# VachaLab/gorder

Measured on AMD Instinct MI355X. Metric: trajectory frames/sec, higher is better.
Workload: dtype f32

## Files before the change

gorder_amd/csrc/gorder_hip.hip:

```cpp
#include <hip/hip_runtime.h>

#include <dlfcn.h>

#include <cmath>
#include <cstdio>
#include <cstdlib>
#include <cstring>
#include <mutex>
#include <new>
#include <string>
#include <deque>
#include <type_traits>
#include <vector>

#include "../../include/gorder_hip.h"
#include "gm_math.h"
#include "plan.h"
#include "collect_store.h"
#include "replay_rows.h"
#include "timewise_blocks.h"
#include "ordermap_final.h"
#include "order_route.h"

#pragma clang fp contract(off)

using gorder::DirectItem;
using gorder::Item;
using gorder::kBlock;
using gorder::Plan;
using gorder::Tile;

#include "kernels_common.h"
#include "kernels_bonds.h"
#include "kernels_extras.h"
#include "kernels_radial.h"
#include "kernels_leaflets.h"
#include "kernels_cluster.h"
#include "kernels_cluster_cutoff.h"
#include "kernels_normals.h"
#include "kernels_xtc.h"
#include "kernels_trr.h"
#include "kernels_collect.h"
#include "kernels_replay.h"
#include "kernels_timewise.h"
#include "kernels_ordermap.h"


struct gorder_hip_handle {
    void *traj_cache = nullptr;
    void (*traj_cache_free)(gorder_hip_handle *) = nullptr;
    Plan plan;
    gorder_tables_t tables{};
    int device = 0;
    hipStream_t own_stream = nullptr;
    hipStream_t stream = nullptr;
// ... 1775 lines not shown
        HIP_TRY(h, hipMalloc((void **)&nc, ncap * row * sizeof(unsigned long long)));
        HIP_TRY(h, hipMemsetAsync(ns, 0, ncap * row * sizeof(unsigned long long), h->stream));
        HIP_TRY(h, hipMemsetAsync(nc, 0, ncap * row * sizeof(unsigned long long), h->stream));
        if (h->d_tw_sums) {
            HIP_TRY(h, hipMemcpyAsync(ns, h->d_tw_sums, h->n_frames * row * sizeof(unsigned long long), hipMemcpyDeviceToDevice, h->stream));
            HIP_TRY(h, hipMemcpyAsync(nc, h->d_tw_cnts, h->n_frames * row * sizeof(unsigned long long), hipMemcpyDeviceToDevice, h->stream));
            HIP_TRY(h, hipStreamSynchronize(h->stream));
            HIP_TRY(h, hipFree(h->d_tw_sums));
            HIP_TRY(h, hipFree(h->d_tw_cnts));
        }
        h->d_tw_sums = ns; h->d_tw_cnts = nc; h->tw_cap = ncap;
    }
    FrameArgs a{};
    a.xyz = d_xyz; a.box9 = d_box; a.n_atoms = p.n_atoms; a.n_frames = n_frames;
    a.pbc = pbc ? 1 : 0;
    a.nx = h->tables.normal[0]; a.ny = h->tables.normal[1]; a.nz = h->tables.normal[2]; a.n2 = h->n2; a.n2sq = h->n2sq;
    a.leaflets = leaflets ? 1 : 0; a.aflags = h->d_aflags; a.arow = h->d_arow; a.n_mol_total = p.n_mol_total;
    a.acc = h->d_acc; a.rep = h->d_rep; a.n_rep = h->n_rep; a.n_acc = p.n_acc; a.err = h->d_err;
    h->manual_active = false;
    if (h->manual_frames) {
        const size_t n4 = (size_t)n_frames * p.n_mol_total;
        if ((st = ensure(h, &h->d_dyn_normals, &h->dyn_normals_cap, n4)) != GORDER_OK) return abort_batch(st);
        if (hipStreamSynchronize(h->stream) != hipSuccess ||
            hipMemcpy(h->d_dyn_normals, h->manual_normals.data(), n4 * 4 * sizeof(float), hipMemcpyHostToDevice) != hipSuccess)
            return abort_batch(fail(h, GORDER_ERR_DEVICE, "manual normals: copy to the device failed"));
        h->manual_active = true;
        h->manual_frames = 0;
    } else if (h->d_ntable) {
        if ((st = replay_normal_rows(h, normal_rows)) != GORDER_OK) return abort_batch(st);
        h->manual_active = true;
    }
    const uint32_t n_tiles_all = (uint32_t)p.tiles.size();
    if (spec) {
        if ((st = ensure(h, &h->d_mom, &h->mom_cap, (size_t)n_frames * n_tiles_all)) != GORDER_OK) return abort_batch(st);
        if ((st = ensure(h, &h->d_head_z, &h->head_z_cap, (size_t)n_frames * p.n_mol_total)) != GORDER_OK) return abort_batch(st);
        a.own = h->d_own; a.mom = h->d_mom; a.mom_dim = (int)lf.normal_dim;
        a.own_head_begin = h->d_own_head_begin; a.own_heads = h->d_own_heads; a.head_z = h->d_head_z;
    }
    h->extra.touched = nullptr;
    if ((h->collect & GORDER_COLLECT_NORMALS) && h->extra.geom_kind && !p.tiles.empty() && p.ua_tiles.empty()) {
        const size_t nt = (size_t)n_frames * p.n_mol_total;
        if ((st = ensure(h, &h->d_touched, &h->touched_cap, nt)) != GORDER_OK) return abort_batch(st);
        if (hipMemsetAsync(h->d_touched, 0, nt, h->stream) != hipSuccess) return abort_batch(fail(h, GORDER_ERR_DEVICE, "collect: hipMemsetAsync"));
        h->extra.touched = h->d_touched;
    }
    st = launch_orders(h, a, route);
    h->manual_active = false;
    if (st != GORDER_OK) return abort_batch(st);
    h->rep_dirty = true;
    if (spec) {
        size_t cap_c = h->spec_frames_cap, cap_o = h->spec_frames_cap;
        if ((st = ensure(h, &h->d_spec_center, &cap_c, n_frames)) != GORDER_OK) return abort_batch(st);
        if ((st = ensure(h, &h->d_spec_ok, &cap_o, n_frames)) != GORDER_OK) return abort_batch(st);
        h->spec_frames_cap = std::min(cap_c, cap_o);
        uint32_t *cnt = h->d_spec_counters + 2u * (uint32_t)(h->spec_batches & 1u);
        uint32_t *cnt_next = h->d_spec_counters + 2u * (uint32_t)((h->spec_batches + 1u) & 1u);
        SpecArgs sa{};
        sa.xyz = d_xyz; sa.box9 = d_box; sa.n_atoms = p.n_atoms; sa.n_frames = n_frames; sa.n_tiles = n_tiles_all;
        sa.n_mol_total = p.n_mol_total; sa.n_membrane = lf.n_membrane; sa.dim = lf.normal_dim; sa.flip = lf.flip ? 1 : 0;
        sa.pbc = pbc ? 1 : 0; sa.mom = h->d_mom; sa.head_z = h->d_head_z; sa.center = h->d_spec_center; sa.ok = h->d_spec_ok;
        sa.aflags = h->d_aflags; sa.adist = h->d_adist; sa.counters = cnt; sa.counters_next = cnt_next;
        const uint32_t ring_slot = (uint32_t)(h->spec_batches % gorder_hip_handle::kSpecRing);
        sa.host_counters = h->h_spec_counters + 2u * ring_slot; sa.err = h->d_err;
        (void)timing_mark(h, "k_spec_check + k_spec_fixup");
        hipLaunchKernelGGL(k_spec_check, dim3(std::min<uint32_t>(n_frames, 2048u)), dim3(256), 0, h->stream, sa);
        if ((st = run_leaflets(h, d_xyz, d_box, spec_aframes, 1, h->d_spec_ok)) != GORDER_OK) return abort_batch(st);
        (void)timing_mark(h, "k_spec_check + k_spec_fixup");
        const uint32_t fix_grid = (uint32_t)std::min<uint64_t>(((uint64_t)n_frames * p.n_mol_total + 63u) / 64u, 4096u);
        with_bool(route.fixup_ac, [&](auto AC) { with_bool(route.fixup_tw, [&](auto TW) {
            if constexpr (!AC() || !TW())
                hipLaunchKernelGGL((k_spec_fixup<AC(), TW()>), dim3(fix_grid), dim3(64), 0, h->stream, a, sa, h->d_spec_mol_begin,
                                   h->d_spec_samples, TW() ? h->d_tw_sums : nullptr, TW() ? h->d_tw_cnts : nullptr,
                                   TW() ? (uint64_t)h->n_frames : (uint64_t)0);
        }); });
        hipLaunchKernelGGL(k_spec_finish, dim3(1), dim3(256), 0, h->stream, sa);
        HIP_TRY(h, hipGetLastError());
        HIP_TRY(h, hipEventRecord(h->spec_counters_copied[ring_slot], h->stream));
        h->spec_ring_frames[ring_slot] = n_frames;
        h->spec_batches++;
    }
    if ((st = collect_flag_rows(h, 1, collect_frames)) != GORDER_OK) return abort_batch(st);
    if (ltable && (h->collect & GORDER_COLLECT_LEAFLETS)) {
        for (size_t k = 0; k < replay.collect_rows.size();) {
            size_t e = k + 1;
            while (e < replay.collect_rows.size() && replay.collect_rows[e] == replay.collect_rows[e - 1] + 1u) e++;
            const std::vector<uint64_t> run(replay.collect_frames.begin() + k, replay.collect_frames.begin() + e);
            if ((st = collect_flag_rows(h, replay.collect_rows[k], run)) != GORDER_OK) return abort_batch(st);
            k = e;
        }
    }
    if ((h->collect & GORDER_COLLECT_NORMALS) && p.n_mol_total && !h->d_ntable &&
        (st = collect_normal_rows(h, frame_index, n_frames, h->extra.touched)) != GORDER_OK) return abort_batch(st);
    if (n_new_rows) {
        HIP_TRY(h, hipMemcpyAsync(h->d_aflags, h->d_aflags + n_new_rows * (size_t)p.n_mol_total, p.n_mol_total,
                                  hipMemcpyDeviceToDevice, h->stream));
    }
    if (ltable) { h->replay_have_carry = replay.have_carry; h->replay_carry_index = replay.carry_index; }
    {
// ... 906 lines not shown
```

gorder_amd/csrc/kernels_bonds.h:

```cpp
#pragma once

namespace {

__device__ __forceinline__ int grid_index(float x, float lo, float bin, uint32_t n, bool core) {
    const float k = __builtin_roundf(core ? gm_div_core(x - lo, bin) : (x - lo) / bin);
    if (!(k >= 0.0f) || !(k < (float)n)) return -1;
    return (int)k;
}
__device__ __forceinline__ int grid_index_fast(float x, float lo, float inv_bin, uint32_t n) {
    const float k = __builtin_floorf(__builtin_fmaf(x - lo, inv_bin, 0.5f));
    if (!(k >= 0.0f) || !(k < (float)n)) return -1;
    return (int)k;
}
constexpr uint32_t kRecFrames = 4;
struct TiledMapOut {
    uint32_t plane;
    float x0, y0, binx, biny;
    uint32_t nx, ny;
    int bin_core;
    unsigned long long *words;
    unsigned long long *ticks;
};
__device__ __forceinline__ unsigned long long tick_sample_word(int tick, bool lower) {
    return ((unsigned long long)(lower ? 1u : 0u) << 32) | (unsigned long long)(uint32_t)tick;
// ... 82 lines not shown
    }
    template <bool TAIL, bool FINITE = false>
    static __device__ __forceinline__ bool store(const FrameArgs &a, const Tile &t, uint32_t f0, uint32_t f_end,
                                                 uint32_t sk, uint32_t si, const v4f (&pre)[NPF], float *lds,
                                                 uint32_t lw) {
        const uint32_t f = f0 + sk;
        if (TAIL && f >= f_end) return true;
        const size_t base = ((size_t)f * a.n_atoms + t.atom0) * 3u;
        const uint32_t n4 = ((uint32_t)(base & 3u) + 3u * t.n_window + 3u) >> 2;
        const v4f *src = reinterpret_cast<const v4f *>(a.xyz + (base & ~(size_t)3));
        v4f *dst = reinterpret_cast<v4f *>(lds + (size_t)sk * lw);
        typedef float v2f __attribute__((ext_vector_type(2)));
        v2f poison = {0.0f, 0.0f};
        const v2f zero2 = {0.0f, 0.0f};
#pragma unroll
        for (int j = 0; j < NPF; j++) {
            const uint32_t i = si + (uint32_t)j * TPF;
            if (i < n4) dst[i] = pre[j];
            if (FINITE) {
                poison = __builtin_elementwise_fma(pre[j].xy, zero2, poison);
                poison = __builtin_elementwise_fma(pre[j].zw, zero2, poison);
            }
        }
        for (uint32_t i = si + (uint32_t)NPF * TPF; i < n4; i += TPF) {
            const v4f v = __builtin_nontemporal_load(src + i);
            dst[i] = v;
            if (FINITE) {
                poison = __builtin_elementwise_fma(v.xy, zero2, poison);
                poison = __builtin_elementwise_fma(v.zw, zero2, poison);
            }
        }
        return poison.x + poison.y == 0.0f;
    }
    template <int NF, int OUT = 0>
    static __device__ __forceinline__ void compute_core(const FrameArgs &a, const Tile &t, const Item &it,
                                                        uint32_t f0, const float (&P)[NF][6], SampleAcc &acc,
                                                        int &bad, uint32_t &nan_which, uint32_t &nan_frame,
                                                        const TiledMapOut *mo = nullptr, uint32_t k0 = 0) {
        constexpr bool MAPS = OUT != 0;
        int tick[NF];
        uint8_t fl[NF];
        float bx[NF], by[NF], bz[NF];
        uint32_t rare = 0;
        auto stage_word = [&](int k, float vx, float vy, float vz) {
            mo->words[k0 + (uint32_t)k] = OUT == 2
                ? tick_sample_word(tick[k], LEAF && fl[k] != 0)
                : map_sample_word(*mo, P[k][0] + vx / 2.0f, P[k][1] + vy / 2.0f, P[k][2] + vz / 2.0f, tick[k], LEAF && fl[k] != 0);
            if (OUT == 3) mo->ticks[k0 + (uint32_t)k] = tick_sample_word(tick[k], LEAF && fl[k] != 0);
        };
#pragma unroll
        for (int k = 0; k < NF; k++) {
            if (PBC) {
                const float *b = a.box9 + 9 * (size_t)(f0 + k);
                bx[k] = b[0]; by[k] = b[4]; bz[k] = b[8];
            }
            if (LEAF) fl[k] = a.aflags[(size_t)a.arow[f0 + k] * a.n_mol_total + it.mol];
        }
#pragma unroll
        for (int k = 0; k < NF; k++) {
            float vx = P[k][3] - P[k][0], vy = P[k][4] - P[k][1], vz = P[k][5] - P[k][2];
            bool slow = false;
            if (PBC && AXIS >= 0 && !ACOS_COS && !MAPS) {
                const float ax = __builtin_fabsf(vx), ay = __builtin_fabsf(vy), az = __builtin_fabsf(vz);
                const float tx = bx[k] - ax, ty = by[k] - ay, tz = bz[k] - az;
                vx = ax > bx[k] / 2.0f ? tx : ax;
                vy = ay > by[k] / 2.0f ? ty : ay;
                vz = az > bz[k] / 2.0f ? tz : az;
                slow = __builtin_fminf(__builtin_fminf(tx, ty), tz) < 0.0f;
            } else if (PBC) {
                vx = gm_min_image_step(vx, bx[k], slow);
                vy = gm_min_image_step(vy, by[k], slow);
                vz = gm_min_image_step(vz, bz[k], slow);
            }
            if (AXIS >= 0 && !ACOS_COS) {
                const float sch = gm_sch_axis<AXIS>(vx, vy, vz, slow);
                rare |= (slow ? 1u : 0u) << k;
                tick[k] = gm_tick_finite(sch);
            } else if (AXIS >= 0) {
                const float sch = gm_sch_axis_acos<AXIS>(vx, vy, vz, slow);
                rare |= (slow ? 1u : 0u) << k;
                tick[k] = gm_tick_finite(sch);
            } else {
                bool nonfinite = false;
                const float sch = gm_calc_sch<ACOS_COS, AXIS>(vx, vy, vz, a.nx, a.ny, a.nz, a.n2, a.n2sq, &nonfinite);
                rare |= ((slow || nonfinite || sch != sch) ? 1u : 0u) << k;
                tick[k] = gm_tick(sch);
            }
            if (MAPS) stage_word(k, vx, vy, vz);
        }
        if (__builtin_expect(rare != 0, 0)) {
#pragma unroll
            for (int k = 0; k < NF; k++) {
                if (!((rare >> k) & 1u)) continue;
                float vx = P[k][3] - P[k][0], vy = P[k][4] - P[k][1], vz = P[k][5] - P[k][2];
                if (PBC) {
                    vx = gm_min_image_loop(vx, bx[k], bad);
                    vy = gm_min_image_loop(vy, by[k], bad);
                    vz = gm_min_image_loop(vz, bz[k], bad);
                }
                const float sch = gm_calc_sch<ACOS_COS>(vx, vy, vz, a.nx, a.ny, a.nz, a.n2, a.n2sq);
                tick[k] = gm_tick(sch);
                if (MAPS) stage_word(k, vx, vy, vz);
                if (sch != sch && nan_frame == kNoNan) {
                    if (P[k][0] != P[k][0]) { nan_which = 0; nan_frame = f0 + k; }
                    else if (P[k][3] != P[k][3]) { nan_which = 1; nan_frame = f0 + k; }
                }
            }
        }
        int st = 0, su = 0;
        uint32_t nu = 0;
#pragma unroll
        for (int k = 0; k < NF; k++) {
            st += tick[k];
            if (LEAF) {
                su += fl[k] == 0 ? tick[k] : 0;
                nu += fl[k] == 0 ? 1u : 0u;
            }
        }
        acc.s_tot += st;
        acc.n_tot += NF;
        acc.s_up += su;
        acc.n_up += nu;
    }
    template <int OUT = 0>
    static __device__ __forceinline__ void compute(const FrameArgs &a, const Tile &t, const Item &it, uint32_t f0,
                                                   const float *lds, uint32_t lw, SampleAcc &acc, int &bad,
                                                   uint32_t &nan_which, uint32_t &nan_frame, const TiledMapOut *mo = nullptr) {
        constexpr int NF = (OUT == 1 || OUT == 3 || (OUT == 2 && LEAF)) ? 2 : (GORDER_COMPUTE_NF < G ? GORDER_COMPUTE_NF : G);
#pragma unroll
        for (int h = 0; h < G; h += NF) {
            float P[NF][6];
#pragma unroll
            for (int k = 0; k < NF; k++) {
                const uint32_t sh = (uint32_t)((((size_t)(f0 + h + k) * a.n_atoms + t.atom0) * 3u) & 3u);
                const float *w = lds + (size_t)(h + k) * lw + sh;
                P[k][0] = w[3u * it.li]; P[k][1] = w[3u * it.li + 1]; P[k][2] = w[3u * it.li + 2];
                P[k][3] = w[3u * it.lj]; P[k][4] = w[3u * it.lj + 1]; P[k][5] = w[3u * it.lj + 2];
            }
            compute_core<NF, OUT>(a, t, it, f0 + h, P, acc, bad, nan_which, nan_frame, mo, (uint32_t)h);
        }
    }
    template <int OUT = 0>
    static __device__ __forceinline__ void compute_tail(const FrameArgs &a, const Tile &t, const Item &it,
                                                        uint32_t f0, uint32_t f_end, const float *lds, uint32_t lw,
                                                        SampleAcc &acc, int &bad, uint32_t &nan_which,
                                                        uint32_t &nan_frame, const TiledMapOut *mo = nullptr) {
        if (OUT != 0) {
#pragma unroll
            for (int k = 0; k < G; k++) {
                const uint32_t f = f0 + (uint32_t)k;
                if (f >= f_end) continue;
                const uint32_t sh = (uint32_t)((((size_t)f * a.n_atoms + t.atom0) * 3u) & 3u);
                const float *w = lds + (size_t)k * lw + sh;
                const float p1x = w[3u * it.li], p1y = w[3u * it.li + 1], p1z = w[3u * it.li + 2];
                const float p2x = w[3u * it.lj], p2y = w[3u * it.lj + 1], p2z = w[3u * it.lj + 2];
                if (bond_sample<ACOS_COS>(a, f, p1x, p1y, p1z, p2x, p2y, p2z, it.mol, acc, bad, mo, mo->words + k, OUT == 3 ? mo->ticks + k : nullptr) &&
                    nan_frame == kNoNan) {
                    if (p1x != p1x) { nan_which = 0; nan_frame = f; }
                    else if (p2x != p2x) { nan_which = 1; nan_frame = f; }
                }
            }
            return;
        }
#pragma unroll 1
        for (uint32_t f = f0; f < f_end; f++) {
            const uint32_t sh = (uint32_t)((((size_t)f * a.n_atoms + t.atom0) * 3u) & 3u);
            const float *w = lds + (size_t)(f - f0) * lw + sh;
            const float p1x = w[3u * it.li], p1y = w[3u * it.li + 1], p1z = w[3u * it.li + 2];
            const float p2x = w[3u * it.lj], p2y = w[3u * it.lj + 1], p2z = w[3u * it.lj + 2];
            if (bond_sample<ACOS_COS>(a, f, p1x, p1y, p1z, p2x, p2y, p2z, it.mol, acc, bad) && nan_frame == kNoNan) {
                if (p1x != p1x) { nan_which = 0; nan_frame = f; }
                else if (p2x != p2x) { nan_which = 1; nan_frame = f; }
            }
        }
    }
};

#ifndef GORDER_TILED_MIN_WAVES
#define GORDER_TILED_MIN_WAVES 4
#endif
__device__ __forceinline__ float mom_min(float x, float y) { float r; __asm__("v_min_f32_e32 %0, %1, %2" : "=v"(r) : "v"(x), "v"(y)); return r; }
__device__ __forceinline__ float mom_max(float x, float y) { float r; __asm__("v_max_f32_e32 %0, %1, %2" : "=v"(r) : "v"(x), "v"(y)); return r; }
#define GORDER_MOM_MINMAX_DPP(CTRL_TEXT)                                                                    \
    __asm__("s_nop 1\n\tv_min_f32_dpp %0, %0, %0 " CTRL_TEXT "\n\tv_max_f32_dpp %1, %1, %1 " CTRL_TEXT : "+v"(mn), "+v"(mx))
__device__ __forceinline__ void tiled_moments(const FrameArgs &a, const Tile &t, uint2 own, uint32_t tile_id, uint32_t n_tiles,
                                              uint32_t f, const float *slot, bool finite, uint2 my_head) {
    const uint32_t lane = threadIdx.x & 63u;
    const uint32_t sh = (uint32_t)((((size_t)f * a.n_atoms + t.atom0) * 3u) & 3u);
    const float *w = slot + sh + a.mom_dim + 3u * (own.x - t.atom0);
    const uint32_t n_own = own.y - own.x;
    float s = 0.0f, q = 0.0f, mn = 3.0e38f, mx = -3.0e38f;
    for (uint32_t i0 = 0; i0 < n_own; i0 += 512u) {
        float z[8];
#pragma unroll
        for (uint32_t u = 0; u < 8u; u++) z[u] = w[3u * min(i0 + 64u * u + lane, n_own - 1u)];
#pragma unroll
        for (uint32_t u = 0; u < 8u; u++) {
            if (i0 + 64u * u >= n_own) break;
            float d = z[u];
            if (i0 + 64u * u + 64u > n_own) d = i0 + 64u * u + lane < n_own ? d : 0.0f;
            s += d;
            q = __builtin_fmaf(d, d, q);
            mn = mom_min(mn, z[u]);
            mx = mom_max(mx, z[u]);
        }
    }
#define GORDER_MOM_STEP(CTRL, MASK, CTRL_TEXT)                                                  \
    s += dpp_or_zero<CTRL, MASK>(s); q += dpp_or_zero<CTRL, MASK>(q);                               \
    GORDER_MOM_MINMAX_DPP(CTRL_TEXT);
    GORDER_MOM_STEP(0x111, 0xf, "row_shr:1 row_mask:0xf bank_mask:0xf")
    GORDER_MOM_STEP(0x112, 0xf, "row_shr:2 row_mask:0xf bank_mask:0xf")
    GORDER_MOM_STEP(0x114, 0xf, "row_shr:4 row_mask:0xf bank_mask:0xf")
    GORDER_MOM_STEP(0x118, 0xf, "row_shr:8 row_mask:0xf bank_mask:0xf")
    GORDER_MOM_STEP(0x142, 0xa, "row_bcast:15 row_mask:0xa bank_mask:0xf")
    GORDER_MOM_STEP(0x143, 0xc, "row_bcast:31 row_mask:0xc bank_mask:0xf")
#undef GORDER_MOM_STEP
    const bool all_finite = __all(finite);
    if (lane == 63u) a.mom[(size_t)f * n_tiles + tile_id] = make_float4(all_finite ? s : __builtin_nanf(""), q, mn, mx);
    if (my_head.y != 0xffffffffu) a.head_z[(size_t)f * a.n_mol_total + my_head.y] = slot[sh + a.mom_dim + 3u * my_head.x];
}
template <int G, int NPF, bool ACOS_COS, bool PBC, bool LEAF, int AXIS, bool MOM = false>
__global__ __launch_bounds__(kBlock, GORDER_TILED_MIN_WAVES) void k_bonds_tiled(FrameArgs a_in, const float *__restrict__ xyz,
                                                      const float *__restrict__ box9,
                                                      const uint8_t *__restrict__ aflags,
                                                      const uint32_t *__restrict__ arow,
                                                      const Tile *__restrict__ tiles,
                                                      const Item *__restrict__ items,
                                                      const uint32_t *__restrict__ tile_slots,
                                                      uint32_t n_tiles, uint32_t lw) {
    extern __shared__ __attribute__((aligned(16))) float lds[];
    using S = TiledStage<G, NPF, ACOS_COS, PBC, LEAF, AXIS>;
    FrameArgs a = a_in;
    a.xyz = xyz; a.box9 = box9; a.aflags = aflags; a.arow = arow;
    const uint32_t tile_id = blockIdx.x % n_tiles;
    const uint32_t chunk = blockIdx.x / n_tiles;
    const Tile t = tiles[tile_id];
    const uint32_t tid = threadIdx.x;
    const uint32_t sk = tid / S::TPF, si = tid % S::TPF;
    const bool active = tid < t.n_items;
    Item it{0, 0, 0, 0, 0};
    if (active) it = items[t.item0 + tid];

    const uint32_t f_begin = chunk * a.frames_per_chunk;
    const uint32_t f_end = min(a.n_frames, f_begin + a.frames_per_chunk);
    const uint32_t f_full = f_begin + ((f_end - f_begin) / G) * G;

    SampleAcc acc;
    int bad = 0;
    uint32_t nan_which = 0, nan_frame = kNoNan;
    v4f pre[NPF];
    uint2 own = make_uint2(0u, 0u), my_head = make_uint2(0u, 0xffffffffu);
    if (MOM) {
        own = a.own[tile_id];
        const uint32_t hq = a.own_head_begin[tile_id] + (tid & 63u);
        if (hq < a.own_head_begin[tile_id + 1u]) my_head = a.own_heads[hq];
    }

    if (f_begin < f_full) S::template load<false>(a, t, f_begin, f_end, sk, si, pre);
    for (uint32_t f0 = f_begin; f0 < f_full; f0 += G) {
        const bool finite = S::template store<false, MOM>(a, t, f0, f_end, sk, si, pre, lds, lw);
        __syncthreads();
        if (f0 + G < f_full) S::template load<false>(a, t, f0 + G, f_end, sk, si, pre);
        if (MOM) {
            static_assert(!MOM || (uint32_t)G * 64u == kBlock, "a wave per frame slot");
            tiled_moments(a, t, own, tile_id, n_tiles, f0 + sk, lds + (size_t)sk * lw, finite, my_head);
        }
        if (active) S::compute(a, t, it, f0, lds, lw, acc, bad, nan_which, nan_frame);
        __syncthreads();
    }
    if (f_full < f_end) {
        S::template load<true>(a, t, f_full, f_end, sk, si, pre);
        const bool finite = S::template store<true, MOM>(a, t, f_full, f_end, sk, si, pre, lds, lw);
        __syncthreads();
        if (MOM && f_full + sk < f_end) tiled_moments(a, t, own, tile_id, n_tiles, f_full + sk, lds + (size_t)sk * lw, finite, my_head);
        if (active) S::compute_tail(a, t, it, f_full, f_end, lds, lw, acc, bad, nan_which, nan_frame);
        __syncthreads();
    }

    if (nan_frame != kNoNan)
        raise_error(a.err, GORDER_ERR_UNDEFINED_POSITION, nan_frame, kStageTypes, tile_slots[t.slot0 + it.lslot], 1, it.mol, nan_which);
    if (bad) raise_box_range(a.err, f_begin);

    unsigned long long *l_s = reinterpret_cast<unsigned long long *>(lds);
    uint32_t *l_n = reinterpret_cast<uint32_t *>(l_s + 2 * kBlock);
    l_s[tid] = 0; l_s[kBlock + tid] = 0; l_n[tid] = 0; l_n[kBlock + tid] = 0;
    __syncthreads();
    if (active && acc.n_tot) {
        atomicAdd(&l_s[it.lslot], (unsigned long long)acc.s_tot);
        atomicAdd(&l_n[it.lslot], acc.n_tot);
        if (acc.n_up) {
            atomicAdd(&l_s[kBlock + it.lslot], (unsigned long long)acc.s_up);
            atomicAdd(&l_n[kBlock + it.lslot], acc.n_up);
        }
    }
    __syncthreads();
#ifdef GORDER_DEBUG_NOEPILOGUE
    if (a.n_frames == 0xffffffffu)
#endif
    if (tid < t.n_slots && l_n[tid]) {
        unsigned long long *acc = a.rep + (size_t)(blockIdx.x % a.n_rep) * 4u * a.n_acc;
        const uint32_t slot = tile_slots[t.slot0 + tid];
        atomicAdd(&acc[slot], l_s[tid]);
        atomicAdd(&acc[2u * a.n_acc + slot], (unsigned long long)l_n[tid]);
        if (l_n[kBlock + tid]) {
            atomicAdd(&acc[a.n_acc + slot], l_s[kBlock + tid]);
            atomicAdd(&acc[3u * a.n_acc + slot], (unsigned long long)l_n[kBlock + tid]);
        }
// ... 128 lines not shown
```

gorder_amd/csrc/kernels_extras.h:

```cpp
#pragma once

namespace {

struct ExtraArgs {
    int maps;
    uint32_t plane;
    float x0, y0, binx, biny;
    uint32_t nx, ny;
    unsigned long long *map_packed;
    unsigned long long *map_rec;
    const uint32_t *item_run;
    uint32_t rec_frame0, rec_stride;
    const float4 *dyn;
    int bin_core;
    float inv_binx, inv_biny;
    int axis;
    int tw;
    unsigned long long *tw_sums;
    unsigned long long *tw_cnts;
    unsigned long long tw_row0;
    float sin_tet, cos_tet, sin_ch3, cos_ch3, sin_half, cos_half;
    int geom_kind, geom_invert, geom_orient;
    float geom_thr;
    const float *shapes;
// ... 325 lines not shown
    __shared__ uint32_t l_slot_run[kBlock];
    __shared__ uint32_t l_slot_id[kBlock];
    using S = TiledStage<G, NPF, false, PBC, LEAF, AXIS>;
    FrameArgs a = a_in;
    a.xyz = xyz; a.box9 = box9; a.aflags = aflags; a.arow = arow;
    const uint32_t tile_id = blockIdx.x % n_tiles, chunk = blockIdx.x / n_tiles;
    const Tile t = tiles[tile_id];
    const uint32_t tid = threadIdx.x;
    const uint32_t sk = tid / S::TPF, si = tid % S::TPF;
    const bool active = tid < t.n_items;
    Item it{0, 0, 0, 0, 0};
    if (active) {
        it = items[t.item0 + tid];
        const uint32_t run = e.item_run[t.item0 + tid];
        if ((run >> 16) == tid) l_slot_run[it.lslot] = run;
    }
    const uint32_t f_begin = a.frame0 + chunk * a.frames_per_chunk;
    const uint32_t f_end = min(a.n_frames, f_begin + a.frames_per_chunk);
    unsigned long long words[kRecFrames], mwords[MAPS ? kRecFrames : 1];
    TiledMapOut mo{};
    if (MAPS) {
        mo.plane = e.plane; mo.x0 = e.x0; mo.y0 = e.y0; mo.binx = e.binx; mo.biny = e.biny; mo.nx = e.nx; mo.ny = e.ny;
        mo.bin_core = e.bin_core; mo.words = mwords; mo.ticks = words;
    } else {
        mo.nx = 0;
        mo.words = words;
    }
    SampleAcc acc;
    int bad = 0;
    uint32_t nan_which = 0, nan_frame = kNoNan;
    v4f pre[NPF];
    const uint32_t my_slot = tid < t.n_slots ? tile_slots[t.slot0 + tid] : 0u;
    l_slot_id[tid] = my_slot;
    uint2 own = make_uint2(0u, 0u), my_head = make_uint2(0u, 0xffffffffu);
    if (MOM) {
        own = a.own[tile_id];
        const uint32_t hq = a.own_head_begin[tile_id] + (tid & 63u);
        if (hq < a.own_head_begin[tile_id + 1u]) my_head = a.own_heads[hq];
    }
    if (f_begin + G <= f_end) S::template load<false>(a, t, f_begin, f_end, sk, si, pre);
    for (uint32_t fs = f_begin; fs < f_end; fs += G) {
        const bool full = fs + G <= f_end;
        bool finite;
        if (full) {
            finite = S::template store<false, MOM>(a, t, fs, f_end, sk, si, pre, lds, lw);
        } else {
            S::template load<true>(a, t, fs, f_end, sk, si, pre);
            finite = S::template store<true, MOM>(a, t, fs, f_end, sk, si, pre, lds, lw);
        }
        __syncthreads();
        if (full && fs + 2u * G <= f_end) S::template load<false>(a, t, fs + G, f_end, sk, si, pre);
        if (MOM && fs + sk < f_end) {
            static_assert(!MOM || (uint32_t)G * 64u == kBlock, "a wave per frame slot");
            tiled_moments(a, t, own, tile_id, n_tiles, fs + sk, lds + (size_t)sk * lw, finite, my_head);
        }
#pragma unroll
        for (uint32_t k = 0; k < kRecFrames; k++) { words[k] = kMapNoSample; if (MAPS) mwords[k] = kMapNoSample; }
        if (active) {
            if (full) S::template compute<MAPS ? 3 : 2>(a, t, it, fs, lds, lw, acc, bad, nan_which, nan_frame, &mo);
            else S::template compute_tail<MAPS ? 3 : 2>(a, t, it, fs, f_end, lds, lw, acc, bad, nan_which, nan_frame, &mo);
        }
        if constexpr (MAPS) rec_store(e, tile_id, fs, tid, mwords);
#pragma unroll
        for (uint32_t k = 0; k < kRecFrames; k++) {
            l_tick[k][tid] = (int)(uint32_t)words[k];
            l_side[k][tid] = words[k] == kMapNoSample ? (uint8_t)2 : (uint8_t)(words[k] >> 32);
        }
        __syncthreads();
        for (uint32_t w = tid; w < kRecFrames * t.n_slots; w += kBlock) {
            const uint32_t k = w % kRecFrames, ls = w / kRecFrames;
            if (fs + k >= f_end) continue;
            const uint32_t run = l_slot_run[ls], tid0 = run >> 16, n = run & 0xffffu;
            int s_all = 0, s_low = 0;
            uint32_t n_all = 0, n_low = 0;
            for (uint32_t j = 0; j < n; j++) {
                const uint32_t side = l_side[k][tid0 + j];
                const int tick = l_tick[k][tid0 + j];
                if (side == 2u) continue;
                s_all += tick; n_all += 1u;
                if (side == 1u) { s_low += tick; n_low += 1u; }
            }
            if (!n_all) continue;
            const uint32_t slot = l_slot_id[ls];
            const size_t row = ((size_t)e.tw_row0 + fs + k) * 3u * a.n_acc;
            atomicAdd(&e.tw_sums[row + slot], (unsigned long long)(long long)s_all);
            atomicAdd(&e.tw_cnts[row + slot], (unsigned long long)n_all);
            if (LEAF) {
                const uint32_t n_up = n_all - n_low;
                if (n_up) {
                    atomicAdd(&e.tw_sums[row + (size_t)a.n_acc + slot], (unsigned long long)(long long)(s_all - s_low));
                    atomicAdd(&e.tw_cnts[row + (size_t)a.n_acc + slot], (unsigned long long)n_up);
                }
// ... 820 lines not shown
```

gorder_amd/csrc/kernels_leaflets.h:

```cpp
#pragma once

namespace {

struct LeafletArgs {
    const float *xyz;
    const float *box9;
    uint32_t n_atoms;
    const uint32_t *aframes;
    uint32_t row0;
    uint8_t *aflags;
    float *adist;
    uint32_t n_mol_total;
    const uint32_t *heads;
    const uint32_t *membrane;
    uint32_t n_membrane;
    const uint32_t *methyl_begin;
    const uint32_t *methyl_atoms;
    uint32_t dim;
    int flip, pbc;
    uint32_t *err;
    const uint8_t *skip;
    uint32_t n_assign;
};

// ... 323 lines not shown
    __syncthreads();
    const float cdim = s_center;
    uint8_t *row = a.aflags + (size_t)(a.row0 + bi) * a.n_mol_total;
    const bool last = bi + 1 == a.n_assign;
    for (uint32_t m = threadIdx.x; m < a.n_mol_total; m += blockDim.x) {
        const float hp = x[3u * (size_t)a.heads[m] + dn];
        float d = hp - cdim;
        if (pbc) d = gm_min_image(d, L, bad);
        row[m] = (uint8_t)((d >= 0.0f ? 0 : 1) ^ (a.flip ? 1 : 0));
        if (last && a.adist) a.adist[m] = d;
    }
    if (bad) raise_box_range(a.err, f);
}
template <bool TURNS>
__global__ __launch_bounds__(256) void k_leaflets_global_contig(LeafletArgs a) {
    if (!TURNS) {
        leaflets_global_contig_frame(a, blockIdx.x);
        return;
    }
    for (uint32_t bi = blockIdx.x; bi < a.n_assign; bi += gridDim.x) {
        leaflets_global_contig_frame(a, bi);
        __syncthreads();
    }
}

struct SpecArgs {
    const float *xyz;
    const float *box9;
    uint32_t n_atoms, n_frames, n_tiles, n_mol_total, n_membrane;
    uint32_t dim;
    int flip, pbc;
    const float4 *mom;
    const float *head_z;
    float *center;
    uint8_t *ok;
    uint8_t *aflags;
    float *adist;
    uint32_t *counters;
    uint32_t *counters_next;
    uint32_t *host_counters;
    uint32_t *err;
};
__global__ __launch_bounds__(256) void k_spec_check(SpecArgs a) {
    __shared__ float s_center;
    __shared__ int s_ok;
    for (uint32_t f = blockIdx.x; f < a.n_frames; f += gridDim.x) {
        const float L = a.pbc ? a.box9[9 * (size_t)f + 4 * a.dim] : 0.0f;
        if (threadIdx.x < 64u) {
            double S = 0.0, Q = 0.0;
            float mn = 3.0e38f, mx = -3.0e38f;
            for (uint32_t t = threadIdx.x; t < a.n_tiles; t += 64u) {
                const float4 m = a.mom[(size_t)f * a.n_tiles + t];
                S += (double)m.x; Q += (double)m.y;
                mn = fminf(mn, m.z); mx = fmaxf(mx, m.w);
            }
            wave_sum2_minmax_bfly(S, Q, mn, mx);
            if (threadIdx.x == 0u) {
                const double n = (double)a.n_membrane, c = S / n;
                bool ok = (S - S == 0.0) && (Q - Q == 0.0) && mn <= mx;
                if (ok && a.pbc) {
                    const double k = 6.283185307179586 / (double)L;
                    const double var = fmax(Q - S * S / n, 0.0) + 1e-4 * Q + 1e-6 * n;
                    const double dmax = k * fmax((double)mx - c, c - (double)mn), S2 = k * k * var, den = n - 0.5 * S2;
                    ok = den > 0.0 && L > 0.0f;
                    if (ok) {
                        const double dist = (dmax * S2 / 6.0 / den) / k;
                        const double room = 0.5 * (double)L - 1e-4 * (double)L - dist;
                        ok = (double)mx - c < room && c - (double)mn < room;
                    }
                }
                a.center[f] = (float)c;
                a.ok[f] = ok ? 1 : 0;
                s_center = (float)c;
                s_ok = ok ? 1 : 0;
                if (!ok) atomicAdd(&a.counters[1], 1u);
            }
        }
        __syncthreads();
        if (s_ok) {
            const float c = s_center;
            const bool last = f + 1 == a.n_frames;
            int bad = 0;
            for (uint32_t m = threadIdx.x; m < a.n_mol_total; m += blockDim.x) {
                float d = a.head_z[(size_t)f * a.n_mol_total + m] - c;
                if (a.pbc) d = gm_min_image(d, L, bad);
                a.aflags[(size_t)(1u + f) * a.n_mol_total + m] = (uint8_t)((d >= 0.0f ? 0 : 1) ^ (a.flip ? 1 : 0));
                if (last && a.adist) a.adist[m] = d;
            }
            if (bad) raise_box_range(a.err, f);
        }
        __syncthreads();
    }
}
struct SpecSample { uint32_t i, j, slot; };
template <bool ACOS_COS, bool TW>
__global__ __launch_bounds__(64) void k_spec_fixup(FrameArgs a, SpecArgs sa, const uint32_t *__restrict__ mol_begin,
                                                   const SpecSample *__restrict__ samples, unsigned long long *tw_sums,
                                                   unsigned long long *tw_cnts, uint64_t tw_row0) {
    const uint64_t n_pairs = (uint64_t)sa.n_frames * sa.n_mol_total;
    uint32_t moved = 0;
    for (uint64_t p0 = (uint64_t)blockIdx.x * 64u; p0 < n_pairs; p0 += (uint64_t)gridDim.x * 64u) {
        const uint64_t pi = p0 + threadIdx.x;
        bool differs = false;
        uint32_t exact_l = 0;
        if (pi < n_pairs) {
            exact_l = sa.aflags[(size_t)sa.n_mol_total + pi];
            differs = exact_l != sa.aflags[pi % sa.n_mol_total];
        }
        unsigned long long todo = __ballot(differs);
        moved += (uint32_t)__popcll(todo);
        while (todo) {
            const int l = __ffsll((long long)todo) - 1;
            todo &= todo - 1ull;
            const uint64_t pj = p0 + (uint64_t)l;
            const uint32_t f = (uint32_t)(pj / sa.n_mol_total), m = (uint32_t)(pj - (uint64_t)f * sa.n_mol_total);
            const uint32_t exact = (uint32_t)__shfl((int)exact_l, l, 64);
            const float *x = a.xyz + (size_t)f * a.n_atoms * 3u;
            for (uint32_t q = mol_begin[m] + threadIdx.x; q < mol_begin[m + 1]; q += 64u) {
                const SpecSample sm = samples[q];
                SampleAcc acc;
                int bad = 0;
                const float *p1 = x + 3u * (size_t)sm.i, *p2 = x + 3u * (size_t)sm.j;
// ... 1588 lines not shown
```

Before: 21.10 million.

## Store speculative leaflet moments tile-major and split center/check into batched kernels

Moments and head z-values move from a frame-major to a tile-major layout padded to 128-byte lines, so each tile wave writes contiguously across frames. The old per-frame k_spec_check is split in two. A new k_spec_center reduces the moments for several frames per wave, and a 2D-grid k_spec_check assigns leaflet flags over batches of frames per tile. The bond kernels also read the leaflet flag once per molecule instead of once per frame in the speculative path. The price is an extra launch plus integer division and indirect own_heads lookups in the check kernel.

New measurement: 20.17 million. -4.4%, worse.

```diff
diff --git a/gorder_amd/csrc/gorder_hip.hip b/gorder_amd/csrc/gorder_hip.hip
--- a/gorder_amd/csrc/gorder_hip.hip
+++ b/gorder_amd/csrc/gorder_hip.hip
@@ -21,6 +21,7 @@
 #include "timewise_blocks.h"
 #include "ordermap_final.h"
 #include "order_route.h"
+#include "spec_layout.h"
 
 #pragma clang fp contract(off)
 
@@ -1862,8 +1863,9 @@
     }
     const uint32_t n_tiles_all = (uint32_t)p.tiles.size();
     if (spec) {
-        if ((st = ensure(h, &h->d_mom, &h->mom_cap, (size_t)n_frames * n_tiles_all)) != GORDER_OK) return abort_batch(st);
-        if ((st = ensure(h, &h->d_head_z, &h->head_z_cap, (size_t)n_frames * p.n_mol_total)) != GORDER_OK) return abort_batch(st);
+        const gorder::SpecLayout sl = gorder::spec_layout(n_frames);
+        if ((st = ensure(h, &h->d_mom, &h->mom_cap, gorder::spec_mom_capacity(sl, n_tiles_all))) != GORDER_OK) return abort_batch(st);
+        if ((st = ensure(h, &h->d_head_z, &h->head_z_cap, gorder::spec_head_capacity(sl, p.n_mol_total))) != GORDER_OK) return abort_batch(st);
         a.own = h->d_own; a.mom = h->d_mom; a.mom_dim = (int)lf.normal_dim;
         a.own_head_begin = h->d_own_head_begin; a.own_heads = h->d_own_heads; a.head_z = h->d_head_z;
     }
@@ -1888,12 +1890,14 @@
         SpecArgs sa{};
         sa.xyz = d_xyz; sa.box9 = d_box; sa.n_atoms = p.n_atoms; sa.n_frames = n_frames; sa.n_tiles = n_tiles_all;
         sa.n_mol_total = p.n_mol_total; sa.n_membrane = lf.n_membrane; sa.dim = lf.normal_dim; sa.flip = lf.flip ? 1 : 0;
-        sa.pbc = pbc ? 1 : 0; sa.mom = h->d_mom; sa.head_z = h->d_head_z; sa.center = h->d_spec_center; sa.ok = h->d_spec_ok;
+        sa.pbc = pbc ? 1 : 0; sa.mom = h->d_mom; sa.head_z = h->d_head_z; sa.own_head_begin = h->d_own_head_begin; sa.own_heads = h->d_own_heads; sa.center = h->d_spec_center; sa.ok = h->d_spec_ok;
         sa.aflags = h->d_aflags; sa.adist = h->d_adist; sa.counters = cnt; sa.counters_next = cnt_next;
         const uint32_t ring_slot = (uint32_t)(h->spec_batches % gorder_hip_handle::kSpecRing);
         sa.host_counters = h->h_spec_counters + 2u * ring_slot; sa.err = h->d_err;
         (void)timing_mark(h, "k_spec_check + k_spec_fixup");
-        hipLaunchKernelGGL(k_spec_check, dim3(std::min<uint32_t>(n_frames, 2048u)), dim3(256), 0, h->stream, sa);
+        hipLaunchKernelGGL(k_spec_center, dim3(std::min<uint32_t>(gorder::ceil_div(n_frames, gorder::kSpecMomPerLine), 8192u)), dim3(64), 0, h->stream, sa);
+        hipLaunchKernelGGL(k_spec_check, dim3(std::min<uint32_t>(gorder::ceil_div(n_frames, gorder::kSpecCheckFrames), 2048u),
+                                              std::min<uint32_t>(gorder::ceil_div(n_tiles_all, 4u), 64u)), dim3(256), 0, h->stream, sa);
         if ((st = run_leaflets(h, d_xyz, d_box, spec_aframes, 1, h->d_spec_ok)) != GORDER_OK) return abort_batch(st);
         (void)timing_mark(h, "k_spec_check + k_spec_fixup");
         const uint32_t fix_grid = (uint32_t)std::min<uint64_t>(((uint64_t)n_frames * p.n_mol_total + 63u) / 64u, 4096u);
diff --git a/gorder_amd/csrc/kernels_bonds.h b/gorder_amd/csrc/kernels_bonds.h
--- a/gorder_amd/csrc/kernels_bonds.h
+++ b/gorder_amd/csrc/kernels_bonds.h
@@ -138,11 +138,11 @@
         }
         return poison.x + poison.y == 0.0f;
     }
-    template <int NF, int OUT = 0>
+    template <int NF, int OUT = 0, bool ONE_FLAG = false>
     static __device__ __forceinline__ void compute_core(const FrameArgs &a, const Tile &t, const Item &it,
                                                         uint32_t f0, const float (&P)[NF][6], SampleAcc &acc,
                                                         int &bad, uint32_t &nan_which, uint32_t &nan_frame,
-                                                        const TiledMapOut *mo = nullptr, uint32_t k0 = 0) {
+                                                        const TiledMapOut *mo = nullptr, uint32_t k0 = 0, uint8_t flag0 = 0) {
         constexpr bool MAPS = OUT != 0;
         int tick[NF];
         uint8_t fl[NF];
@@ -160,7 +160,7 @@
                 const float *b = a.box9 + 9 * (size_t)(f0 + k);
                 bx[k] = b[0]; by[k] = b[4]; bz[k] = b[8];
             }
-            if (LEAF) fl[k] = a.aflags[(size_t)a.arow[f0 + k] * a.n_mol_total + it.mol];
+            if (LEAF) fl[k] = ONE_FLAG ? flag0 : a.aflags[(size_t)a.arow[f0 + k] * a.n_mol_total + it.mol];
         }
 #pragma unroll
         for (int k = 0; k < NF; k++) {
@@ -218,20 +218,25 @@
 #pragma unroll
         for (int k = 0; k < NF; k++) {
             st += tick[k];
-            if (LEAF) {
+            if (LEAF && !ONE_FLAG) {
                 su += fl[k] == 0 ? tick[k] : 0;
                 nu += fl[k] == 0 ? 1u : 0u;
             }
+        }
+        if (LEAF && ONE_FLAG) {
+            su = flag0 == 0 ? st : 0;
+            nu = flag0 == 0 ? (uint32_t)NF : 0u;
         }
         acc.s_tot += st;
         acc.n_tot += NF;
         acc.s_up += su;
         acc.n_up += nu;
     }
-    template <int OUT = 0>
+    template <int OUT = 0, bool ONE_FLAG = false>
     static __device__ __forceinline__ void compute(const FrameArgs &a, const Tile &t, const Item &it, uint32_t f0,
                                                    const float *lds, uint32_t lw, SampleAcc &acc, int &bad,
-                                                   uint32_t &nan_which, uint32_t &nan_frame, const TiledMapOut *mo = nullptr) {
+                                                   uint32_t &nan_which, uint32_t &nan_frame, const TiledMapOut *mo = nullptr,
+                                                   uint8_t flag0 = 0) {
         constexpr int NF = (OUT == 1 || OUT == 3 || (OUT == 2 && LEAF)) ? 2 : (GORDER_COMPUTE_NF < G ? GORDER_COMPUTE_NF : G);
 #pragma unroll
         for (int h = 0; h < G; h += NF) {
@@ -243,7 +248,7 @@
                 P[k][0] = w[3u * it.li]; P[k][1] = w[3u * it.li + 1]; P[k][2] = w[3u * it.li + 2];
                 P[k][3] = w[3u * it.lj]; P[k][4] = w[3u * it.lj + 1]; P[k][5] = w[3u * it.lj + 2];
             }
-            compute_core<NF, OUT>(a, t, it, f0 + h, P, acc, bad, nan_which, nan_frame, mo, (uint32_t)h);
+            compute_core<NF, OUT, ONE_FLAG>(a, t, it, f0 + h, P, acc, bad, nan_which, nan_frame, mo, (uint32_t)h, flag0);
         }
     }
     template <int OUT = 0>
@@ -289,8 +294,8 @@
 __device__ __forceinline__ float mom_max(float x, float y) { float r; __asm__("v_max_f32_e32 %0, %1, %2" : "=v"(r) : "v"(x), "v"(y)); return r; }
 #define GORDER_MOM_MINMAX_DPP(CTRL_TEXT)                                                                    \
     __asm__("s_nop 1\n\tv_min_f32_dpp %0, %0, %0 " CTRL_TEXT "\n\tv_max_f32_dpp %1, %1, %1 " CTRL_TEXT : "+v"(mn), "+v"(mx))
-__device__ __forceinline__ void tiled_moments(const FrameArgs &a, const Tile &t, uint2 own, uint32_t tile_id, uint32_t n_tiles,
-                                              uint32_t f, const float *slot, bool finite, uint2 my_head) {
+__device__ __forceinline__ void tiled_moments(const FrameArgs &a, const Tile &t, uint2 own, uint32_t tile_id, const gorder::SpecLayout &sl,
+                                              uint32_t f, const float *slot, bool finite, uint2 my_head, uint2 head_row) {
     const uint32_t lane = threadIdx.x & 63u;
     const uint32_t sh = (uint32_t)((((size_t)f * a.n_atoms + t.atom0) * 3u) & 3u);
     const float *w = slot + sh + a.mom_dim + 3u * (own.x - t.atom0);
@@ -311,6 +316,10 @@
             mx = mom_max(mx, z[u]);
         }
     }
+#ifdef GORDER_DEBUG_SPEC_NOREDUCE
+    if (a.n_frames == 0xffffffffu) a.mom[lane] = make_float4(finite ? s : q, q, mn, mx);
+    return;
+#endif
 #define GORDER_MOM_STEP(CTRL, MASK, CTRL_TEXT)                                                  \
     s += dpp_or_zero<CTRL, MASK>(s); q += dpp_or_zero<CTRL, MASK>(q);                               \
     GORDER_MOM_MINMAX_DPP(CTRL_TEXT);
@@ -322,8 +331,11 @@
     GORDER_MOM_STEP(0x143, 0xc, "row_bcast:31 row_mask:0xc bank_mask:0xf")
 #undef GORDER_MOM_STEP
     const bool all_finite = __all(finite);
-    if (lane == 63u) a.mom[(size_t)f * n_tiles + tile_id] = make_float4(all_finite ? s : __builtin_nanf(""), q, mn, mx);
-    if (my_head.y != 0xffffffffu) a.head_z[(size_t)f * a.n_mol_total + my_head.y] = slot[sh + a.mom_dim + 3u * my_head.x];
+#ifdef GORDER_DEBUG_SPEC_NOSTORE
+    if (a.n_frames != 0xffffffffu) return;
+#endif
+    if (lane == 63u) a.mom[gorder::spec_mom_index(sl, tile_id, f)] = make_float4(all_finite ? s : __builtin_nanf(""), q, mn, mx);
+    if (my_head.y != 0xffffffffu) a.head_z[gorder::spec_head_index(sl, head_row.x, head_row.y, lane, f)] = slot[sh + a.mom_dim + 3u * my_head.x];
 }
 template <int G, int NPF, bool ACOS_COS, bool PBC, bool LEAF, int AXIS, bool MOM = false>
 __global__ __launch_bounds__(kBlock, GORDER_TILED_MIN_WAVES) void k_bonds_tiled(FrameArgs a_in, const float *__restrict__ xyz,
@@ -355,11 +367,15 @@
     int bad = 0;
     uint32_t nan_which = 0, nan_frame = kNoNan;
     v4f pre[NPF];
-    uint2 own = make_uint2(0u, 0u), my_head = make_uint2(0u, 0xffffffffu);
+    uint2 own = make_uint2(0u, 0u), my_head = make_uint2(0u, 0xffffffffu), head_row = make_uint2(0u, 0u);
+    uint8_t flag0 = 0;
+    const gorder::SpecLayout sl = gorder::spec_layout(MOM ? a.n_frames : 0u);
     if (MOM) {
         own = a.own[tile_id];
-        const uint32_t hq = a.own_head_begin[tile_id] + (tid & 63u);
-        if (hq < a.own_head_begin[tile_id + 1u]) my_head = a.own_heads[hq];
+        const uint32_t q0 = a.own_head_begin[tile_id], q1 = a.own_head_begin[tile_id + 1u], hq = q0 + (tid & 63u);
+        if (hq < q1) my_head = a.own_heads[hq];
+        head_row = make_uint2(q0, q1 - q0);
+        if (active) flag0 = a.aflags[it.mol];
     }
 
     if (f_begin < f_full) S::template load<false>(a, t, f_begin, f_end, sk, si, pre);
@@ -369,16 +385,16 @@
         if (f0 + G < f_full) S::template load<false>(a, t, f0 + G, f_end, sk, si, pre);
         if (MOM) {
             static_assert(!MOM || (uint32_t)G * 64u == kBlock, "a wave per frame slot");
-            tiled_moments(a, t, own, tile_id, n_tiles, f0 + sk, lds + (size_t)sk * lw, finite, my_head);
-        }
-        if (active) S::compute(a, t, it, f0, lds, lw, acc, bad, nan_which, nan_frame);
+            tiled_moments(a, t, own, tile_id, sl, f0 + sk, lds + (size_t)sk * lw, finite, my_head, head_row);
+        }
+        if (active) S::template compute<0, MOM>(a, t, it, f0, lds, lw, acc, bad, nan_which, nan_frame, nullptr, flag0);
         __syncthreads();
     }
     if (f_full < f_end) {
         S::template load<true>(a, t, f_full, f_end, sk, si, pre);
         const bool finite = S::template store<true, MOM>(a, t, f_full, f_end, sk, si, pre, lds, lw);
         __syncthreads();
-        if (MOM && f_full + sk < f_end) tiled_moments(a, t, own, tile_id, n_tiles, f_full + sk, lds + (size_t)sk * lw, finite, my_head);
+        if (MOM && f_full + sk < f_end) tiled_moments(a, t, own, tile_id, sl, f_full + sk, lds + (size_t)sk * lw, finite, my_head, head_row);
         if (active) S::compute_tail(a, t, it, f_full, f_end, lds, lw, acc, bad, nan_which, nan_frame);
         __syncthreads();
     }
diff --git a/gorder_amd/csrc/kernels_extras.h b/gorder_amd/csrc/kernels_extras.h
--- a/gorder_amd/csrc/kernels_extras.h
+++ b/gorder_amd/csrc/kernels_extras.h
@@ -381,11 +381,15 @@
     v4f pre[NPF];
     const uint32_t my_slot = tid < t.n_slots ? tile_slots[t.slot0 + tid] : 0u;
     l_slot_id[tid] = my_slot;
-    uint2 own = make_uint2(0u, 0u), my_head = make_uint2(0u, 0xffffffffu);
+    uint2 own = make_uint2(0u, 0u), my_head = make_uint2(0u, 0xffffffffu), head_row = make_uint2(0u, 0u);
+    uint8_t flag0 = 0;
+    const gorder::SpecLayout sl = gorder::spec_layout(MOM ? a.n_frames : 0u);
     if (MOM) {
         own = a.own[tile_id];
-        const uint32_t hq = a.own_head_begin[tile_id] + (tid & 63u);
-        if (hq < a.own_head_begin[tile_id + 1u]) my_head = a.own_heads[hq];
+        const uint32_t q0 = a.own_head_begin[tile_id], q1 = a.own_head_begin[tile_id + 1u], hq = q0 + (tid & 63u);
+        if (hq < q1) my_head = a.own_heads[hq];
+        head_row = make_uint2(q0, q1 - q0);
+        if (active) flag0 = a.aflags[it.mol];
     }
     if (f_begin + G <= f_end) S::template load<false>(a, t, f_begin, f_end, sk, si, pre);
     for (uint32_t fs = f_begin; fs < f_end; fs += G) {
@@ -401,12 +405,12 @@
         if (full && fs + 2u * G <= f_end) S::template load<false>(a, t, fs + G, f_end, sk, si, pre);
         if (MOM && fs + sk < f_end) {
             static_assert(!MOM || (uint32_t)G * 64u == kBlock, "a wave per frame slot");
-            tiled_moments(a, t, own, tile_id, n_tiles, fs + sk, lds + (size_t)sk * lw, finite, my_head);
+            tiled_moments(a, t, own, tile_id, sl, fs + sk, lds + (size_t)sk * lw, finite, my_head, head_row);
         }
 #pragma unroll
         for (uint32_t k = 0; k < kRecFrames; k++) { words[k] = kMapNoSample; if (MAPS) mwords[k] = kMapNoSample; }
         if (active) {
-            if (full) S::template compute<MAPS ? 3 : 2>(a, t, it, fs, lds, lw, acc, bad, nan_which, nan_frame, &mo);
+            if (full) S::template compute<MAPS ? 3 : 2, MOM>(a, t, it, fs, lds, lw, acc, bad, nan_which, nan_frame, &mo, flag0);
             else S::template compute_tail<MAPS ? 3 : 2>(a, t, it, fs, f_end, lds, lw, acc, bad, nan_which, nan_frame, &mo);
         }
         if constexpr (MAPS) rec_store(e, tile_id, fs, tid, mwords);
diff --git a/gorder_amd/csrc/kernels_leaflets.h b/gorder_amd/csrc/kernels_leaflets.h
--- a/gorder_amd/csrc/kernels_leaflets.h
+++ b/gorder_amd/csrc/kernels_leaflets.h
@@ -379,6 +379,8 @@
     int flip, pbc;
     const float4 *mom;
     const float *head_z;
+    const uint32_t *own_head_begin;
+    const uint2 *own_heads;
     float *center;
     uint8_t *ok;
     uint8_t *aflags;
@@ -388,53 +390,99 @@
     uint32_t *host_counters;
     uint32_t *err;
 };
+__device__ __forceinline__ bool spec_center(const SpecArgs &a, float L, double S, double Q, float mn, float mx, float &center) {
+    const double n = (double)a.n_membrane, c = S / n;
+    bool ok = (S - S == 0.0) && (Q - Q == 0.0) && mn <= mx;
+    if (ok && a.pbc) {
+        const double k = 6.283185307179586 / (double)L;
+        const double var = fmax(Q - S * S / n, 0.0) + 1e-4 * Q + 1e-6 * n;
+        const double dmax = k * fmax((double)mx - c, c - (double)mn), S2 = k * k * var, den = n - 0.5 * S2;
+        ok = den > 0.0 && L > 0.0f;
+        if (ok) {
+            const double dist = (dmax * S2 / 6.0 / den) / k;
+            const double room = 0.5 * (double)L - 1e-4 * (double)L - dist;
+            ok = (double)mx - c < room && c - (double)mn < room;
+        }
+    }
+    center = (float)c;
+    return ok;
+}
+__global__ __launch_bounds__(64) void k_spec_center(SpecArgs a) {
+    constexpr uint32_t W = gorder::kSpecMomPerLine;
+    const gorder::SpecLayout sl = gorder::spec_layout(a.n_frames);
+    const uint32_t lane = threadIdx.x;
+    for (uint32_t fw = blockIdx.x * W; fw < a.n_frames; fw += gridDim.x * W) {
+        double S[W], Q[W];
+        float mn[W], mx[W];
+#pragma unroll
+        for (uint32_t k = 0; k < W; k++) { S[k] = 0.0; Q[k] = 0.0; mn[k] = 3.0e38f; mx[k] = -3.0e38f; }
+        for (uint32_t t = lane; t < a.n_tiles; t += 64u) {
+            const float4 *row = a.mom + gorder::spec_mom_index(sl, t, fw);
+#pragma unroll
+            for (uint32_t k = 0; k < W; k++) {
+                const float4 m = row[k];
+                S[k] += (double)m.x; Q[k] += (double)m.y;
+                mn[k] = fminf(mn[k], m.z); mx[k] = fmaxf(mx[k], m.w);
+            }
+        }
+        double my_S = 0.0, my_Q = 0.0;
+        float my_mn = 0.0f, my_mx = 0.0f;
+#pragma unroll
+        for (uint32_t k = 0; k < W; k++) {
+            wave_sum2_minmax_bfly(S[k], Q[k], mn[k], mx[k]);
+            if (lane == k) { my_S = S[k]; my_Q = Q[k]; my_mn = mn[k]; my_mx = mx[k]; }
+        }
+        const uint32_t f = fw + lane;
+        if (lane < W && f < a.n_frames) {
+            const float L = a.pbc ? a.box9[9 * (size_t)f + 4 * a.dim] : 0.0f;
+            float c;
+            const bool ok = spec_center(a, L, my_S, my_Q, my_mn, my_mx, c);
+            a.center[f] = c;
+            a.ok[f] = ok ? 1 : 0;
+            if (!ok) atomicAdd(&a.counters[1], 1u);
+        }
+    }
+}
 __global__ __launch_bounds__(256) void k_spec_check(SpecArgs a) {
-    __shared__ float s_center;
-    __shared__ int s_ok;
-    for (uint32_t f = blockIdx.x; f < a.n_frames; f += gridDim.x) {
-        const float L = a.pbc ? a.box9[9 * (size_t)f + 4 * a.dim] : 0.0f;
-        if (threadIdx.x < 64u) {
-            double S = 0.0, Q = 0.0;
-            float mn = 3.0e38f, mx = -3.0e38f;
-            for (uint32_t t = threadIdx.x; t < a.n_tiles; t += 64u) {
-                const float4 m = a.mom[(size_t)f * a.n_tiles + t];
-                S += (double)m.x; Q += (double)m.y;
-                mn = fminf(mn, m.z); mx = fmaxf(mx, m.w);
-            }
-            wave_sum2_minmax_bfly(S, Q, mn, mx);
-            if (threadIdx.x == 0u) {
-                const double n = (double)a.n_membrane, c = S / n;
-                bool ok = (S - S == 0.0) && (Q - Q == 0.0) && mn <= mx;
-                if (ok && a.pbc) {
-                    const double k = 6.283185307179586 / (double)L;
-                    const double var = fmax(Q - S * S / n, 0.0) + 1e-4 * Q + 1e-6 * n;
-                    const double dmax = k * fmax((double)mx - c, c - (double)mn), S2 = k * k * var, den = n - 0.5 * S2;
-                    ok = den > 0.0 && L > 0.0f;
-                    if (ok) {
-                        const double dist = (dmax * S2 / 6.0 / den) / k;
-                        const double room = 0.5 * (double)L - 1e-4 * (double)L - dist;
-                        ok = (double)mx - c < room && c - (double)mn < room;
-                    }
+    constexpr uint32_t B = gorder::kSpecCheckFrames, U = 4;
+    __shared__ float s_center[B], s_L[B];
+    __shared__ int s_ok[B];
+    const gorder::SpecLayout sl = gorder::spec_layout(a.n_frames);
+    const uint32_t lane = threadIdx.x & 63u, wave = threadIdx.x >> 6;
+    for (uint32_t fb = blockIdx.x * B; fb < a.n_frames; fb += gridDim.x * B) {
+        const uint32_t n_f = min(B, a.n_frames - fb);
+        if (threadIdx.x < B) {
+            const uint32_t f = fb + threadIdx.x;
+            const bool in = threadIdx.x < n_f;
+            s_ok[threadIdx.x] = in ? (int)a.ok[f] : 0;
+            s_center[threadIdx.x] = in ? a.center[f] : 0.0f;
+            s_L[threadIdx.x] = in && a.pbc ? a.box9[9 * (size_t)f + 4 * a.dim] : 0.0f;
+        }
+        __syncthreads();
+        for (uint32_t t = blockIdx.y * 4u + wave; t < a.n_tiles; t += 4u * gridDim.y) {
+            const uint32_t q0 = a.own_head_begin[t], n_heads = a.own_head_begin[t + 1u] - q0, n = n_f * n_heads;
+            const float *row = a.head_z + gorder::spec_head_index(sl, q0, n_heads, 0u, fb);
+            for (uint32_t e0 = lane; e0 < n; e0 += 64u * U) {
+                float z[U];
+                uint32_t r[U], m[U];
+#pragma unroll
+                for (uint32_t u = 0; u < U; u++) {
+                    const uint32_t e = e0 + 64u * u < n ? e0 + 64u * u : 0u;
+                    r[u] = e / n_heads;
+                    z[u] = row[e];
+                    m[u] = a.own_heads[q0 + (e - r[u] * n_heads)].y;
                 }
-                a.center[f] = (float)c;
-                a.ok[f] = ok ? 1 : 0;
-                s_center = (float)c;
-                s_ok = ok ? 1 : 0;
-                if (!ok) atomicAdd(&a.counters[1], 1u);
-            }
-        }
-        __syncthreads();
-        if (s_ok) {
-            const float c = s_center;
-            const bool last = f + 1 == a.n_frames;
-            int bad = 0;
-            for (uint32_t m = threadIdx.x; m < a.n_mol_total; m += blockDim.x) {
-                float d = a.head_z[(size_t)f * a.n_mol_total + m] - c;
-                if (a.pbc) d = gm_min_image(d, L, bad);
-                a.aflags[(size_t)(1u + f) * a.n_mol_total + m] = (uint8_t)((d >= 0.0f ? 0 : 1) ^ (a.flip ? 1 : 0));
-                if (last && a.adist) a.adist[m] = d;
-            }
-            if (bad) raise_box_range(a.err, f);
+#pragma unroll
+                for (uint32_t u = 0; u < U; u++) {
+                    if (e0 + 64u * u >= n || !s_ok[r[u]]) continue;
+                    int bad = 0;
+                    float d = z[u] - s_center[r[u]];
+                    if (a.pbc) d = gm_min_image(d, s_L[r[u]], bad);
+                    a.aflags[(size_t)(1u + fb + r[u]) * a.n_mol_total + m[u]] = (uint8_t)((d >= 0.0f ? 0 : 1) ^ (a.flip ? 1 : 0));
+                    if (fb + r[u] + 1u == a.n_frames && a.adist) a.adist[m[u]] = d;
+                    if (bad) raise_box_range(a.err, fb + r[u]);
+                }
+            }
         }
         __syncthreads();
     }
diff --git a/gorder_amd/csrc/spec_layout.h b/gorder_amd/csrc/spec_layout.h
--- /dev/null
+++ b/gorder_amd/csrc/spec_layout.h
@@ -0,0 +1,41 @@
+#ifndef GORDER_SPEC_LAYOUT_H
+#define GORDER_SPEC_LAYOUT_H
+#include <stddef.h>
+#include <stdint.h>
+
+#if defined(__HIPCC__) || defined(__CUDACC__)
+#define GORDER_SPEC_HD __host__ __device__
+#else
+#define GORDER_SPEC_HD
+#endif
+
+namespace gorder {
+constexpr uint32_t kSpecLineBytes = 128;
+constexpr uint32_t kSpecMomPerLine = kSpecLineBytes / 16u;
+constexpr uint32_t kSpecHeadPerLine = kSpecLineBytes / 4u;
+constexpr uint32_t kSpecCheckFrames = kSpecHeadPerLine;
+
+struct SpecLayout {
+    uint32_t n_frames, n_partials;
+    uint32_t mom_stride;
+    uint32_t head_stride;
+};
+
+GORDER_SPEC_HD inline SpecLayout spec_layout(uint32_t n_frames, uint32_t n_partials = 1) {
+    SpecLayout l;
+    l.n_frames = n_frames; l.n_partials = n_partials;
+    l.mom_stride = (n_frames * n_partials + kSpecMomPerLine - 1u) / kSpecMomPerLine * kSpecMomPerLine;
+    l.head_stride = (n_frames + kSpecHeadPerLine - 1u) / kSpecHeadPerLine * kSpecHeadPerLine;
+    return l;
+}
+GORDER_SPEC_HD inline size_t spec_mom_index(const SpecLayout &l, uint32_t tile, uint32_t frame, uint32_t partial = 0) {
+    return (size_t)tile * l.mom_stride + (size_t)frame * l.n_partials + partial;
+}
+GORDER_SPEC_HD inline size_t spec_mom_capacity(const SpecLayout &l, uint32_t n_tiles) { return (size_t)n_tiles * l.mom_stride; }
+GORDER_SPEC_HD inline size_t spec_head_index(const SpecLayout &l, uint32_t slot0, uint32_t n_heads, uint32_t head, uint32_t frame) {
+    return (size_t)slot0 * l.head_stride + (size_t)frame * n_heads + head;
+}
+GORDER_SPEC_HD inline size_t spec_head_capacity(const SpecLayout &l, uint32_t n_slots) { return (size_t)n_slots * l.head_stride; }
+
+}
+#endif
```
